# PengjieRen/CaSE_RG

Measured on AMD Instinct MI355X. Metric: train tokens/sec (query+passage) CaSE model, higher is better.
Workload: dtype bf16; 1 GPU; CaSE train step fwd+bwd+allreduce+clip+Adam+EMA, d_model=512, 6 encoder layers, 10 passages x 384 tok, query 64, answer 40, vocab 30522, per-GPU batch 32, dropout on; global_batch=32, parallelism=dp1

## Files before the change

case_rg_amd/_abi.py:

```python
import ctypes as C
import os

import torch

_HERE = os.path.dirname(os.path.abspath(__file__))
LIB_PATH = os.environ.get("CASE_HIP_LIB") or os.path.join(_HERE, "csrc", "libcase_hip.so")

ABI_VERSION = 600
F32, BF16 = 0, 1
WS_ATTENTION_SPLITKV, WS_ATTENTION_BWD, WS_OPTIM_SUMSQ, WS_ENCODER_CHAIN_PACK, WS_GEMM_DW_SLABS = 1, 2, 3, 4, 5
(FEAT_GEMM_256, FEAT_GEMM_SMALL, FEAT_ENCODER_CHAIN, FEAT_ATTN_SCORES, FEAT_ATTN_DECODE, FEAT_OPTIM, FEAT_ATTN_RESIDENT, FEAT_RESERVED_CUS,
 FEAT_GEMM_DW_SLABS, FEAT_DECODER_CHAIN, FEAT_ATTN_DECODE_MQA, FEAT_POINTER_DECODE, FEAT_POINTER_HEAD, FEAT_GEMM_LN, FEAT_STEP_STATE,
 FEAT_INTERACTION, FEAT_ATTN_DECODE_APPEND, FEAT_LINEAR_SKINNY, FEAT_BEAM_DECODE, FEAT_SAMPLE_DECODE, FEAT_POINTER_SCORE, FEAT_CONSENSUS, FEAT_NGRAM_BAN,
 FEAT_NGRAM_COUNTS, FEAT_RANK_METRICS, FEAT_POINTER_HEAD_WIDE, FEAT_DECODE_RULES, FEAT_TOKEN_LABELS,
 FEAT_COPY_ATTRIBUTION, FEAT_METEOR, FEAT_RISK_TRAIN, FEAT_ROUGE_N) = (1 << i for i in range(32))
EPI_BIAS_COL, EPI_BIAS_ROW, EPI_GELU, EPI_RELU = 1, 2, 4, 8
EPI_RESIDUAL, EPI_MUL_DGELU, EPI_MUL_DRELU, EPI_ATOMIC, EPI_DROPOUT = 16, 32, 64, 128, 256

i32, i64, u64, f32, f64, ptr = C.c_int32, C.c_int64, C.c_uint64, C.c_float, C.c_double, C.c_void_p


class GemmDesc(C.Structure):
    _fields_ = [(n, i64) for n in ("M", "N", "K", "lda", "ldb", "ldc", "ld_aux", "batch1", "batch2",
                                   "sa1", "sa2", "sb1", "sb2", "sc1", "sc2", "saux1", "saux2")] + \
# ... 86 lines not shown
    "case_nll_gather_bwd": [ptr, ptr, ptr, ptr, i64, i64, ptr],
    "case_row_argmax": [ptr, ptr, ptr, i64, i64, i64, ptr],
    "case_sentence_compact": [ptr, ptr, ptr, i64, i64, i64, i64, i64, ptr],
    "case_encoder_chain_pack": [ptr, ptr, ptr, ptr, ptr, ptr],
    "case_encoder_chain": [C.POINTER(EncoderChainDesc)] + [ptr] * 14,
    "case_set_reserved_cus": [i32],
    "case_attention_decode_mqa": [ptr, ptr, ptr, ptr, i64, i64, i64, i32, ptr, i64, ptr],
    "case_additive_key_exp": [ptr, ptr, i64, ptr],
    "case_pointer_attend_decode": [ptr] * 11 + [i64, i64, i64, ptr],
    "case_pointer_head_decode": [ptr] * 5 + [i32] + [ptr] * 4 + [i64, i64, i64, ptr],
    "case_pointer_head_beam": [ptr] * 5 + [i32] + [ptr] * 4 + [i64, i64, i64, i32, ptr],
    "case_pointer_head_sample": [ptr] * 5 + [i32] + [ptr] * 7 + [i64, i64, i64, f32, i32, f32, u64, u64, ptr, i64, i64, i64, i32, i32, ptr],
    "case_pointer_head_decode_wide": [ptr] * 5 + [i32] + [ptr] * 4 + [i64, i64, i64, ptr, i64, ptr, i64, i64, i32, i64, ptr],
    "case_pointer_head_beam_wide": [ptr] * 5 + [i32] + [ptr] * 4 + [i64, i64, i64, i32, ptr, i64, ptr, i64, i64, i32, i64, ptr],
    "case_pointer_head_sample_wide": [ptr] * 5 + [i32] + [ptr] * 7 + [i64, i64, i64, f32, i32, f32, u64, u64, ptr, i64, i64, i64, i32, i32,
                                      ptr, i64, ptr, i64, i64, i32, ptr],
    "case_pointer_head_score": [ptr] * 3 + [i64, ptr, ptr, i32, ptr, i64, ptr, ptr, i64, i64, i64, ptr],
    "case_beam_advance": [ptr] * 12 + [i64, i64, i64, i32, i64, ptr],
    "case_pointer_head_decode_ban": [ptr] * 5 + [i32] + [ptr] * 4 + [i64, i64, i64, ptr, i64, i64, i32, i64, ptr],
    "case_pointer_head_beam_ban": [ptr] * 5 + [i32] + [ptr] * 4 + [i64, i64, i64, i32, ptr, i64, i64, i32, i64, ptr],
    "case_pointer_head_sample_ban": [ptr] * 5 + [i32] + [ptr] * 7 + [i64, i64, i64, f32, i32, f32, u64, u64, ptr, i64, i64, i64, i32, i32,
                                     ptr, i64, i64, i32, ptr],
    "case_beam_advance_ban": [ptr] * 12 + [i64, i64, i64, i32, i64, ptr, ptr, i64, ptr],
    "case_ngram_ban": [ptr, ptr, ptr, i64, i64, i64, i64, i32, i64, ptr],
    "case_remove_duplicate_ids": [ptr, ptr, i64, i64, i32, i64, ptr],
    "case_pointer_head_decode_rules": [ptr] * 5 + [i32] + [ptr] * 4 + [i64, i64, i64, ptr, i64, i64, i32, i64] + _RULE + [ptr],
    "case_pointer_head_beam_rules": [ptr] * 5 + [i32] + [ptr] * 4 + [i64, i64, i64, i32, ptr, i64, i64, i32, i64] + _RULE + [ptr],
    "case_pointer_head_sample_rules": [ptr] * 5 + [i32] + [ptr] * 7 + [i64, i64, i64, f32, i32, f32, u64, u64, ptr, i64, i64, i64, i32, i32,
                                       ptr, i64, i64, i32] + _RULE + [ptr],
    "case_pointer_head_decode_wide_rules": [ptr] * 5 + [i32] + [ptr] * 4 + [i64, i64, i64, ptr, i64, ptr, i64, i64, i32, i64] + _RULE + [ptr],
    "case_pointer_head_beam_wide_rules": [ptr] * 5 + [i32] + [ptr] * 4 + [i64, i64, i64, i32, ptr, i64, ptr, i64, i64, i32, i64] + _RULE + [ptr],
    "case_pointer_head_sample_wide_rules": [ptr] * 5 + [i32] + [ptr] * 7 + [i64, i64, i64, f32, i32, f32, u64, u64, ptr, i64, i64, i64, i32, i32,
                                            ptr, i64, ptr, i64, i64, i32] + _RULE + [ptr],
    "case_row_rules": [ptr, ptr, i64, i64, i64] + _RULE + [ptr],
    "case_beam_advance_rules": [ptr] * 12 + [i64, i64, i64, i32, i64, ptr, ptr, i64, f32, ptr],
    "case_beam_gather": [ptr, ptr, i32, ptr, ptr, ptr, i64, i32, i64, i64, i64, ptr],
    "case_beam_backtrack": [ptr] * 8 + [i64, i32, i64, ptr],
    "case_lcs_pairs": [ptr] * 6 + [i64, i64, i64, i64, i64, ptr],
    "case_consensus_pick": [ptr] * 7 + [i64, i64, i64, ptr],
    "case_ngram_counts": [ptr] * 9 + [i64, i64, i64, i64, i64, i32, ptr],
    "case_bleu_scores": [ptr] * 7 + [i64, i64, i64, i32, i32, ptr],
    "case_ngram_distinct": [ptr, ptr, ptr, i64, i64, i32, ptr],
    "case_rouge_n_scores": [ptr] * 9 + [i64, i64, i64, i32, ptr],
    "case_rank_metrics": [ptr] * 8 + [i64, i64, i64, ptr],
    "case_token_labels": [ptr, ptr, ptr, i32, ptr, ptr, i64, i64, i64, i64, i64, i64, ptr],
    "case_token_select": [ptr] * 7 + [i64, i64, i32, ptr],
    "case_copy_attribution": [ptr, ptr, i64, ptr, ptr, i32, ptr, i64, ptr, ptr, i32, ptr, ptr, ptr, ptr, i64, i64, i64, ptr],
    "case_meteor": [ptr] * 5 + [i64, f64, f64, f64] + [ptr] * 5 + [i64, i64, i64, i64, i64, ptr],
    "case_pointer_head_score_stats": [ptr] * 3 + [i64, ptr, ptr, i32, ptr, i64, ptr, ptr, ptr, i64, i64, i64, ptr],
    "case_pointer_head_score_bwd": [ptr] * 3 + [i64, ptr, ptr, i32, ptr, i64] + [ptr] * 6 + [i64, i64, i64, ptr],
    "case_sequence_risk": [ptr] * 4 + [f64] + [ptr] * 3 + [i64, i64, i64, ptr],
    "case_pointer_head_loss": [ptr, i64, ptr, ptr, i64, ptr, ptr, i32, ptr, i64, ptr, ptr, ptr, ptr, i64, i64, i64, ptr],
    "case_pointer_head_loss_bwd": [ptr, i64, ptr, ptr, i64, ptr, ptr, i32, ptr, i64, ptr, ptr, ptr, ptr, i32, ptr, ptr, i64, i64, i64, ptr],
    "case_gemm_ln": [C.POINTER(GemmDesc), ptr, ptr, ptr, f32, ptr, ptr, ptr, ptr, ptr, ptr],
    "case_optim_sumsq": [ptr, ptr, i64, ptr, ptr, ptr],
    "case_optim_adam_ema": [ptr, ptr, i64, ptr, f32, f64, f64, f64, f64, ptr, ptr],
    "case_step_advance": [ptr, u64, f64, f64, ptr],
    "case_interaction_supported": [C.POINTER(InteractionDesc)],
    "case_interaction_fwd": [C.POINTER(InteractionDesc), ptr, ptr, ptr, ptr, ptr, ptr, ptr, ptr, ptr, ptr],
}

OPTIONAL = ("case_pointer_head_loss", "case_pointer_head_loss_bwd")


def _load():
    if not os.path.exists(LIB_PATH):
        raise ImportError(
            "case_rg_amd: %s is missing. Build it with `python -c 'import __graft_entry__ as g; g.build()'` "
            "(or `make -C case_rg_amd/csrc`). There is no CPU or eager fallback." % LIB_PATH)
    lib = C.CDLL(LIB_PATH)
    lib.case_version.restype = C.c_int
    if lib.case_version() != ABI_VERSION:
        raise ImportError("case_rg_amd: %s is ABI generation %d, this package binds %d -- rebuild it (make -C case_rg_amd/csrc)"
                          % (LIB_PATH, lib.case_version(), ABI_VERSION))
    for name, args in SIGNATURES.items():
        if name in OPTIONAL and not hasattr(lib, name):
            continue
        fn = getattr(lib, name)
        fn.argtypes = args
        fn.restype = C.c_int
    lib.case_optim_chunk_elems.restype = C.c_int
    lib.case_optim_chunk_elems.argtypes = []
    lib.case_encoder_chain_packed_bytes.restype = C.c_int64
    lib.case_encoder_chain_packed_bytes.argtypes = []
    lib.case_attention_bwd_scratch_floats.restype = C.c_int64
    lib.case_attention_bwd_scratch_floats.argtypes = [C.POINTER(AttnDesc)]
    lib.case_attention_decode_mqa_workspace.restype = C.c_int64
    lib.case_attention_decode_mqa_workspace.argtypes = [i64, i64, i32]
    lib.case_attention_decode_mqa_splits.restype = C.c_int32
    lib.case_attention_decode_mqa_splits.argtypes = [i64, i64]
    lib.case_abi_features.restype = C.c_uint32
    lib.case_abi_features.argtypes = []
    lib.case_get_reserved_cus.restype = C.c_int
    lib.case_get_reserved_cus.argtypes = []
    lib.case_sizeof_opt_tensor.restype = C.c_int
    lib.case_sizeof_opt_tensor.argtypes = []
    lib.case_sizeof_step_state.restype = C.c_int
    lib.case_sizeof_step_state.argtypes = []
    if lib.case_sizeof_step_state() != C.sizeof(StepState):
        raise ImportError("case_rg_amd: CaseStepState is %d bytes in %s, %d in this binding" % (lib.case_sizeof_step_state(), LIB_PATH, C.sizeof(StepState)))
    lib.case_gemm_dw_slab_bytes.restype = C.c_int64
    lib.case_gemm_dw_slab_bytes.argtypes = [C.POINTER(GemmDesc)]
    lib.case_workspace_bytes.restype = C.c_int64
    lib.case_workspace_bytes.argtypes = [i32, ptr, i64]
    lib.case_gemm_tile_for.restype = C.c_int
    lib.case_gemm_tile_for.argtypes = [C.POINTER(GemmDesc), ptr, ptr, ptr, ptr, ptr, ptr]
    lib.case_last_error.restype = C.c_char_p
    return lib


lib = _load()


def has(name):
    return hasattr(lib, name)
# ... 10 lines not shown
```

case_rg_amd/csrc/attn_pointer.hip:

```cpp
#include "common.h"

namespace {

template <bool FAST>
__device__ __forceinline__ float tanh_t(float x) {
  if constexpr (FAST) {
    const float e = __expf(2.f * x);
    return 1.f - __fdividef(2.f, e + 1.f);
  } else {
    return tanhf(x);
  }
}

constexpr float TANH_PRESCALE = 2.8853900817779268f;
constexpr float EXP2_CLAMP = 62.f;
__device__ __forceinline__ float exp2_factor(float xs) { return __builtin_amdgcn_exp2f(fminf(fmaxf(xs, -EXP2_CLAMP), EXP2_CLAMP)); }
__device__ __forceinline__ float half_sigmoid_prod(float ew, float eu) { return __builtin_amdgcn_rcpf(fmaf(ew, eu, 1.f)); }

constexpr int AJ = 64;
constexpr int AH = 64;
constexpr int ATW = 8;

template <typename T, bool FAST>
__global__ __launch_bounds__(256) void additive_fwd_kernel(const float* __restrict__ wq, const T* __restrict__ uh,
// ... 46 lines not shown
        const int64_t t = tc + wave * ATW + i;
        if (t < Tn) s[(b * Tn + t) * S + j] = FAST ? vsum - 2.f * acc[i] : acc[i];
      }
    }
  }
}

template <typename T, bool FAST, int TT, int NCH>
__global__ __launch_bounds__(256) void additive_fwd_rowwise_kernel(const float* __restrict__ wq, const T* __restrict__ uh,
                                                                   const float* __restrict__ v, float* __restrict__ s,
                                                                   int64_t Tn, int64_t S, int64_t H) {
  constexpr int E = Vec16<T>::N;
  const int64_t b = blockIdx.y;
  const int lane = threadIdx.x & 63;
  const int64_t wave = (int64_t)blockIdx.x * 4 + (threadIdx.x >> 6), nwaves = (int64_t)gridDim.x * 4;
  float wreg[NCH][TT][E], vreg[NCH][E];
#pragma unroll
  for (int c = 0; c < NCH; ++c) {
    const int64_t h0 = ((int64_t)c * 64 + lane) * E;
#pragma unroll
    for (int e = 0; e < E; ++e) {
      vreg[c][e] = h0 < H ? v[h0 + e] : 0.f;
#pragma unroll
      for (int t = 0; t < TT; ++t) wreg[c][t][e] = (h0 < H && t < Tn) ? wq[(b * Tn + t) * H + h0 + e] : 0.f;
    }
  }
  for (int64_t j = wave; j < S; j += nwaves) {
    float acc[TT];
#pragma unroll
    for (int t = 0; t < TT; ++t) acc[t] = 0.f;
#pragma unroll
    for (int c = 0; c < NCH; ++c) {
      const int64_t h0 = ((int64_t)c * 64 + lane) * E;
      if (h0 < H) {
        float u[E];
        Vec16<T>::load(uh + (b * S + j) * H + h0, u);
#pragma unroll
        for (int e = 0; e < E; ++e)
#pragma unroll
          for (int t = 0; t < TT; ++t) acc[t] += vreg[c][e] * tanh_t<FAST>(wreg[c][t][e] + u[e]);
      }
    }
#pragma unroll
    for (int t = 0; t < TT; ++t) {
      const float r = wave_sum(acc[t]);
      if (lane == 0 && t < Tn) s[(b * Tn + t) * S + j] = r;
    }
  }
}

constexpr int BJ = 16;
constexpr int BTC = 32;

template <typename T, bool FAST>
__global__ __launch_bounds__(256) void additive_bwd_uh_kernel(const float* __restrict__ ds, const float* __restrict__ wq,
                                                              const T* __restrict__ uh, const float* __restrict__ v,
                                                              float* __restrict__ d_uh, float* __restrict__ d_v, int64_t Tn,
                                                              int64_t S, int64_t H) {
  __shared__ float DS[BTC][BJ];
  const int64_t b = blockIdx.z, j0 = (int64_t)blockIdx.x * BJ, h = (int64_t)blockIdx.y * 256 + threadIdx.x;
  const bool h_ok = h < H;
  float u[BJ], acc[BJ];
#pragma unroll
  for (int jj = 0; jj < BJ; ++jj) {
    const int64_t j = j0 + jj;
    u[jj] = (h_ok && j < S) ? (FAST ? TANH_PRESCALE : 1.f) * Elem<T>::ld(uh + (b * S + j) * H + h) : 0.f;
    if constexpr (FAST) u[jj] = exp2_factor(u[jj]);
    acc[jj] = 0.f;
  }
  float dv = 0.f, gsum = 0.f;
  for (int64_t tc = 0; tc < Tn; tc += BTC) {
    __syncthreads();
    for (int e = threadIdx.x; e < BTC * BJ; e += 256) {
      const int tt = e / BJ, jj = e % BJ;
      const int64_t t = tc + tt, j = j0 + jj;
      DS[tt][jj] = (t < Tn && j < S) ? ds[(b * Tn + t) * S + j] : 0.f;
    }
    __syncthreads();
    const int tmax = (int)((Tn - tc) < BTC ? (Tn - tc) : BTC);
    for (int tt = 0; tt < tmax; ++tt) {
      float w = h_ok ? (FAST ? TANH_PRESCALE : 1.f) * wq[(b * Tn + tc + tt) * H + h] : 0.f;
      if constexpr (FAST) w = exp2_factor(w);
#pragma unroll
      for (int jj = 0; jj < BJ; ++jj) {
        const float g = DS[tt][jj];
        if constexpr (FAST) {
          const float r = half_sigmoid_prod(w, u[jj]);
          const float gr = g * r;
          acc[jj] += gr - gr * r;
          dv += gr;
          gsum += g;
        } else {
          const float th = tanh_t<FAST>(w + u[jj]);
          acc[jj] += g * (1.f - th * th);
          dv += g * th;
        }
      }
    }
  }
  if (h_ok) {
    const float vh = FAST ? 4.f * v[h] : v[h];
#pragma unroll
    for (int jj = 0; jj < BJ; ++jj) {
      const int64_t j = j0 + jj;
      if (j < S) d_uh[(b * S + j) * H + h] = vh * acc[jj];
    }
    atomicAdd(d_v + h, FAST ? gsum - 2.f * dv : dv);
  }
}

constexpr int CT = 8;
constexpr int CJC = 64;

template <typename T, bool FAST>
__global__ __launch_bounds__(256) void additive_bwd_wq_kernel(const float* __restrict__ ds, const float* __restrict__ wq,
                                                              const T* __restrict__ uh, const float* __restrict__ v,
                                                              float* __restrict__ d_wq, int64_t Tn, int64_t S, int64_t H,
                                                              int tblocks, int64_t j_per) {
  __shared__ float DS[CT][CJC];
  const int64_t b = blockIdx.z, t0 = (int64_t)(blockIdx.x % tblocks) * CT, h = (int64_t)blockIdx.y * 256 + threadIdx.x;
  const int64_t j_begin = (int64_t)(blockIdx.x / tblocks) * j_per, j_end = (j_begin + j_per < S) ? j_begin + j_per : S;
  const bool split = j_per < S;
  const bool h_ok = h < H;
  float w[CT], acc[CT];
#pragma unroll
  for (int tt = 0; tt < CT; ++tt) {
    const int64_t t = t0 + tt;
    w[tt] = (h_ok && t < Tn) ? (FAST ? TANH_PRESCALE : 1.f) * wq[(b * Tn + t) * H + h] : 0.f;
    if constexpr (FAST) w[tt] = exp2_factor(w[tt]);
    acc[tt] = 0.f;
  }
  for (int64_t jc = j_begin; jc < j_end; jc += CJC) {
    __syncthreads();
    for (int e = threadIdx.x; e < CT * CJC; e += 256) {
      const int tt = e / CJC, jj = e % CJC;
      const int64_t t = t0 + tt, j = jc + jj;
      DS[tt][jj] = (t < Tn && j < j_end) ? ds[(b * Tn + t) * S + j] : 0.f;
    }
    __syncthreads();
    const int jmax = (int)((j_end - jc) < CJC ? (j_end - jc) : CJC);
    for (int jj = 0; jj < jmax; ++jj) {
      float u = h_ok ? (FAST ? TANH_PRESCALE : 1.f) * Elem<T>::ld(uh + (b * S + jc + jj) * H + h) : 0.f;
      if constexpr (FAST) u = exp2_factor(u);
#pragma unroll
      for (int tt = 0; tt < CT; ++tt) {
        if constexpr (FAST) {
          const float r = half_sigmoid_prod(w[tt], u);
          const float gr = DS[tt][jj] * r;
          acc[tt] += gr - gr * r;
        } else {
          const float th = tanh_t<FAST>(w[tt] + u);
          acc[tt] += DS[tt][jj] * (1.f - th * th);
        }
      }
    }
  }
  if (h_ok) {
    const float vh = FAST ? 4.f * v[h] : v[h];
#pragma unroll
    for (int tt = 0; tt < CT; ++tt) {
      const int64_t t = t0 + tt;
      if (t < Tn) {
        if (split) atomicAdd(d_wq + (b * Tn + t) * H + h, vh * acc[tt]);
        else d_wq[(b * Tn + t) * H + h] = vh * acc[tt];
      }
    }
  }
}

constexpr float EXP_CLAMP = 43.f;
constexpr int PA_WAVES = 16, PA_H = 512;

__global__ __launch_bounds__(256) void additive_key_exp_kernel(const float* __restrict__ uh, bf16_t* __restrict__ eu, int64_t n8) {
  for (int64_t i = (int64_t)blockIdx.x * 256 + threadIdx.x; i < n8; i += (int64_t)gridDim.x * 256) {
    const float4 a = reinterpret_cast<const float4*>(uh)[2 * i], b = reinterpret_cast<const float4*>(uh)[2 * i + 1];
    const float x[8] = {a.x, a.y, a.z, a.w, b.x, b.y, b.z, b.w};
    float y[8];
#pragma unroll
    for (int e = 0; e < 8; ++e) y[e] = __expf(fminf(fmaxf(2.f * x[e], -EXP_CLAMP), EXP_CLAMP));
    Vec16<bf16_t>::store(eu + 8 * i, y);
  }
}

__device__ __forceinline__ float row_sum4(float r0, float r1, float r2, float r3) {
  const auto a = __builtin_amdgcn_permlane32_swap(__float_as_uint(r0), __float_as_uint(r2), false, false);
  const auto b = __builtin_amdgcn_permlane32_swap(__float_as_uint(r1), __float_as_uint(r3), false, false);
  const float A = __uint_as_float(a[0]) + __uint_as_float(a[1]);
  const float B = __uint_as_float(b[0]) + __uint_as_float(b[1]);
  const auto c = __builtin_amdgcn_permlane16_swap(__float_as_uint(A), __float_as_uint(B), false, false);
  float t = __uint_as_float(c[0]) + __uint_as_float(c[1]);
  t += __uint_as_float(__builtin_amdgcn_update_dpp(0, __float_as_uint(t), 0x128, 0xf, 0xf, false));
  t += __uint_as_float(__builtin_amdgcn_update_dpp(0, __float_as_uint(t), 0x124, 0xf, 0xf, false));
  t += __uint_as_float(__builtin_amdgcn_update_dpp(0, __float_as_uint(t), 0x122, 0xf, 0xf, false));
  t += __uint_as_float(__builtin_amdgcn_update_dpp(0, __float_as_uint(t), 0x121, 0xf, 0xf, false));
  return t;
}

#ifndef CASE_STREAM_DEFAULT_POLICY
typedef unsigned int pa_u32x4 __attribute__((ext_vector_type(4)));
__device__ __forceinline__ uint4 pa_nt_load(const void* p) {
  const pa_u32x4 v = __builtin_nontemporal_load(reinterpret_cast<const pa_u32x4*>(p));
  return make_uint4(v[0], v[1], v[2], v[3]);
}
#define PA_STREAM_LOAD(P) pa_nt_load(P)
#else
#define PA_STREAM_LOAD(P) (*reinterpret_cast<const uint4*>(P))
#endif
__global__ __launch_bounds__(64 * PA_WAVES) void pointer_attend_decode_kernel(
    const float* __restrict__ wq, const float* __restrict__ wq_add, const bf16_t* __restrict__ eu, const float* __restrict__ v, const bf16_t* __restrict__ mem,
    const uint8_t* __restrict__ col_valid, const uint8_t* __restrict__ row_valid, const float* __restrict__ prior, bf16_t* __restrict__ ctx,
    float* __restrict__ p_out, float* __restrict__ copy_out, const int64_t S) {
  extern __shared__ __attribute__((aligned(16))) float pa_smem[];
  float* sc = pa_smem;
  float* red = pa_smem + ((S + 3) & ~(int64_t)3);
  const int lane = threadIdx.x & 63, wave = threadIdx.x >> 6;
  const int64_t b = blockIdx.x;
  const uint8_t* cv = col_valid ? col_valid + b * S : nullptr;
  const bool row_ok = row_valid ? row_valid[b] != 0 : true;
  float ew[8], vv[8];
// ... 1175 lines not shown
                                        int64_t S, int64_t H, int32_t dtype, case_stream_t stream) {
  CASE_REQUIRE(wq && uh && v && s && B > 0 && T > 0 && S > 0 && H > 0 && B < 65536, "case_additive_scores_fwd: bad argument");
  hipStream_t st = (hipStream_t)stream;
  const int ev = dtype == CASE_F32 ? 4 : 8;
  if (T <= 2 && H % ev == 0 && H <= 2 * 64 * ev && (uintptr_t)uh % 16 == 0) {
    const dim3 g((unsigned)((S + 15) / 16 < 64 ? (S + 15) / 16 : 64), (unsigned)B);
    const bool one = H <= 64 * ev;
#define ROWWISE(TY, FAST, TT, NCH) hipLaunchKernelGGL((additive_fwd_rowwise_kernel<TY, FAST, TT, NCH>), g, dim3(256), 0, st, wq, (const TY*)uh, v, s, T, S, H)
    if (dtype == CASE_F32) {
      if (T == 1) { if (one) ROWWISE(float, false, 1, 1); else ROWWISE(float, false, 1, 2); }
      else { if (one) ROWWISE(float, false, 2, 1); else ROWWISE(float, false, 2, 2); }
    } else {
      if (T == 1) { if (one) ROWWISE(bf16_t, true, 1, 1); else ROWWISE(bf16_t, true, 1, 2); }
      else { if (one) ROWWISE(bf16_t, true, 2, 1); else ROWWISE(bf16_t, true, 2, 2); }
    }
#undef ROWWISE
    return case_check_launch("case_additive_scores_fwd");
  }
  const int64_t jb = (S + AJ - 1) / AJ, tchunks = (T + 4 * ATW - 1) / (4 * ATW);
  const dim3 grid((unsigned)jb, (unsigned)B, (unsigned)(jb * B < 512 ? tchunks : 1));
  if (dtype == CASE_F32)
    hipLaunchKernelGGL((additive_fwd_kernel<float, false>), grid, dim3(256), 0, st, wq, (const float*)uh, v, s, T, S, H);
  else
    hipLaunchKernelGGL((additive_fwd_kernel<bf16_t, true>), grid, dim3(256), 0, st, wq, (const bf16_t*)uh, v, s, T, S, H);
  return case_check_launch("case_additive_scores_fwd");
}

extern "C" int case_additive_scores_bwd(const float* ds, const float* wq, const void* uh, const float* v, float* d_wq,
                                        float* d_uh, float* d_v, int64_t B, int64_t T, int64_t S, int64_t H, int32_t dtype,
                                        case_stream_t stream) {
  CASE_REQUIRE(ds && wq && uh && v && d_wq && d_uh && d_v && B > 0 && T > 0 && S > 0 && H > 0 && B < 65536,
               "case_additive_scores_bwd: bad argument");
  const unsigned hb = (unsigned)((H + 255) / 256);
  const int tblocks = (int)((T + CT - 1) / CT);
  const int64_t base_wgs = (int64_t)tblocks * hb * B, j_chunks = (S + CJC - 1) / CJC;
  int64_t sch = base_wgs >= 2048 ? 1 : (2048 + base_wgs - 1) / base_wgs;
  if (sch > j_chunks) sch = j_chunks;
  const int64_t j_per = ((j_chunks + sch - 1) / sch) * CJC;
  sch = (S + j_per - 1) / j_per;
  const dim3 g1((unsigned)((S + BJ - 1) / BJ), hb, (unsigned)B), g2((unsigned)(tblocks * sch), hb, (unsigned)B);
  hipStream_t st = (hipStream_t)stream;
  if (sch > 1 && hipMemsetAsync(d_wq, 0, (size_t)(B * T * H) * sizeof(float), st) != hipSuccess)
    return case_set_error(CASE_E_LAUNCH, "case_additive_scores_bwd: hipMemsetAsync failed");
  if (dtype == CASE_F32) {
    hipLaunchKernelGGL((additive_bwd_uh_kernel<float, false>), g1, dim3(256), 0, st, ds, wq, (const float*)uh, v, d_uh, d_v, T, S, H);
    hipLaunchKernelGGL((additive_bwd_wq_kernel<float, false>), g2, dim3(256), 0, st, ds, wq, (const float*)uh, v, d_wq, T, S, H, tblocks, j_per);
  } else {
    hipLaunchKernelGGL((additive_bwd_uh_kernel<bf16_t, true>), g1, dim3(256), 0, st, ds, wq, (const bf16_t*)uh, v, d_uh, d_v, T, S, H);
    hipLaunchKernelGGL((additive_bwd_wq_kernel<bf16_t, true>), g2, dim3(256), 0, st, ds, wq, (const bf16_t*)uh, v, d_wq, T, S, H, tblocks, j_per);
  }
  return case_check_launch("case_additive_scores_bwd");
}

extern "C" int case_additive_key_exp(const float* uh, void* eu, int64_t n, case_stream_t stream) {
  CASE_REQUIRE(uh && eu && n > 0 && n % 8 == 0 && (uintptr_t)uh % 16 == 0 && (uintptr_t)eu % 16 == 0, "case_additive_key_exp: bad argument");
  hipLaunchKernelGGL(additive_key_exp_kernel, dim3(grid_for(n / 8, 256, 1, 256 * 32)), dim3(256), 0, (hipStream_t)stream, uh,
                     reinterpret_cast<bf16_t*>(eu), n / 8);
  return case_check_launch("case_additive_key_exp");
}

extern "C" int case_pointer_attend_decode(const float* wq, const float* wq_add, const void* eu, const float* v, const void* value, const uint8_t* col_valid,
                                          const uint8_t* row_valid, const float* prior, void* ctx, float* p, float* copy, int64_t B, int64_t S,
                                          int64_t H, case_stream_t stream) {
  CASE_REQUIRE(wq && eu && v && value && ctx && p && B > 0 && S > 0 && B < (1ll << 31) && (copy != nullptr) == (prior != nullptr),
               "case_pointer_attend_decode: bad argument");
  if (H != PA_H || S > 28000)
    return case_set_error(CASE_E_UNSUPPORTED, "case_pointer_attend_decode: built for H = %d and S <= 28000 (run case_additive_scores_fwd + "
                                              "case_softmax_fwd + case_gemm)", PA_H);
  for (const void* q : {(const void*)wq, (const void*)wq_add, eu, (const void*)v, value})
    CASE_REQUIRE((reinterpret_cast<uintptr_t>(q) & 15) == 0, "case_pointer_attend_decode: tensors must be 16-byte aligned");
  const size_t lds = (size_t)(((S + 3) & ~(int64_t)3) + PA_WAVES * PA_H) * sizeof(float);
  static bool attr = false;
  if (!attr) {
    if (hipFuncSetAttribute(reinterpret_cast<const void*>(&pointer_attend_decode_kernel), hipFuncAttributeMaxDynamicSharedMemorySize, 160 * 1024) !=
        hipSuccess)
      return case_set_error(CASE_E_LAUNCH, "case_pointer_attend_decode: cannot reserve LDS");
    attr = true;
  }
  hipLaunchKernelGGL(pointer_attend_decode_kernel, dim3((unsigned)B), dim3(64 * PA_WAVES), lds, (hipStream_t)stream, wq, wq_add,
                     reinterpret_cast<const bf16_t*>(eu), v, reinterpret_cast<const bf16_t*>(value), col_valid, row_valid, prior,
                     reinterpret_cast<bf16_t*>(ctx), p, copy, S);
  return case_check_launch("case_pointer_attend_decode");
}

template <typename Args>
static int pointer_head_fill(Args& a, const char* who, const float* logits, const float* mix_logits, const uint32_t* keys, const float* const* copies,
                             const int64_t* lens, int32_t nmem, int64_t R, int64_t V, int64_t S, int64_t max_v, const char* instead) {
  CASE_REQUIRE(logits && mix_logits && keys && copies && lens && R > 0 && V > 0 && S > 0 && nmem >= 1 && R < (1ll << 31), "%s: bad argument", who);
  if (nmem > PH_MAX_MEM || V > max_v || S > 32768)
    return case_set_error(CASE_E_UNSUPPORTED, "%s: built for <= %d memories, V <= %lld, S <= 32768%s", who, PH_MAX_MEM, (long long)max_v, instead);
  a.logits = logits;
  a.mix_logits = mix_logits;
  a.keys = keys;
  int64_t total = 0;
  for (int m = 0; m < PH_MAX_MEM; ++m) {
    a.copy[m] = m < nmem ? copies[m] : nullptr;
    a.len[m] = m < nmem ? lens[m] : 0;
    total += a.len[m];
    CASE_REQUIRE(m >= nmem || (copies[m] && lens[m] > 0), "%s: null copy weights", who);
  }
  CASE_REQUIRE(total == S, "%s: the memories hold %lld positions, the source map %lld", who, (long long)total, (long long)S);
  a.V = V;
  a.S = S;
  a.nmem = nmem;
  return CASE_OK;
}
// ... 673 lines not shown
```

case_rg_amd/ops.py:

```python
import collections
import math
import ctypes as C
import os

import torch
from torch.autograd import Function

from . import _abi as A
from . import config, paramcache

_DT = {torch.float32: A.F32, torch.bfloat16: A.BF16}


def _code(t):
    try:
        return _DT[t.dtype]
    except KeyError:
        raise TypeError("case_rg_amd: unsupported activation dtype %s" % t.dtype)


_raw_stream, _cur_device = getattr(torch._C, "_cuda_getCurrentRawStream", None), getattr(torch._C, "_cuda_getDevice", None)


def _stream():
# ... 1552 lines not shown
        dEpw = bg(dU, Eqx, Lp, H, Lq, Lq, H, yk=True)
        epw = torch.empty_like(Ep3)
        A.call("case_scale_cols", _ptr(Ep3), _ptr(w3), _ptr(epw), n * Lp, H, _code(Ep3), st)
        dEq_parts.append(bg(dU, epw, Lq, H, Lp, Lq, H, xk=True, yk=True))
        dEp_s = torch.empty_like(Ep3)
        dw1, dw2, dw3 = _zeros_like_shapes(dev, (H,), (H,), (H,))
        A.call("case_scale_cols_bwd", _ptr(dEpw), _ptr(Ep3), _ptr(w3), _ptr(dEp_s), _ptr(dw3), n * Lp, H, _code(Ep3), st)
        dEp_parts.append(dEp_s)
        dap, dcq = dU32.sum(dim=2).reshape(-1).contiguous(), dU32.sum(dim=1).reshape(-1).contiguous()
        dEp_r, dEq_r = torch.empty_like(Ep3), torch.empty_like(Eqx)
        A.call("case_rowdot_bwd", _ptr(dap), _ptr(Ep3), _ptr(w2), _ptr(dEp_r), _ptr(dw2), None, n * Lp, H, _code(Ep3), st)
        A.call("case_rowdot_bwd", _ptr(dcq), _ptr(Eqx), _ptr(w1), _ptr(dEq_r), _ptr(dw1), None, n * Lq, H, _code(Eqx), st)
        dEp_parts.append(dEp_r)
        dEq_parts.append(dEq_r)
        dEp = add_n(dEp_parts).view(Ep.shape)
        dEq = add_n(dEq_parts).view(B, P, Lq, H)
        if nq != P:
            dEq = dEq.float().sum(dim=1, keepdim=True).to(dt)
        dw = torch.cat([dw1, dw2, dw3]).view(w.shape)
        return dEq, dEp, dw, None, None


def interaction_train_supported(Eq, Ep):
    return INTERACTION_TRAIN and interaction_supported(Eq, Ep, False)


class MaxOverPFn(Function):
    @staticmethod
    def forward(ctx, x):
        B, P = x.shape[0], x.shape[1]
        x = x if x.is_contiguous() else x.contiguous()
        inner = x.numel() // (B * P)
        out = torch.empty(B, 1, *x.shape[2:], dtype=x.dtype, device=x.device)
        arg = torch.empty(B * inner, dtype=torch.int32, device=x.device)
        A.call("case_max_over_p_fwd", _ptr(x), _ptr(out), _ptr(arg), B, P, inner, _code(x), _stream())
        ctx.save_for_backward(arg)
        ctx.shape = x.shape
        return out

    @staticmethod
    def backward(ctx, g):
        (arg,) = ctx.saved_tensors
        B, P = ctx.shape[0], ctx.shape[1]
        g = g if g.is_contiguous() else g.contiguous()
        dx = torch.empty(ctx.shape, dtype=g.dtype, device=g.device)
        A.call("case_max_over_p_bwd", _ptr(g), _ptr(arg), _ptr(dx), B, P, dx.numel() // (B * P), _code(g), _stream())
        return dx


def max_over_p(x):
    return MaxOverPFn.apply(x)


class AdditiveScoresFn(Function):
    @staticmethod
    def forward(ctx, wq, uh, v):
        B, T, H = wq.shape
        S = uh.shape[1]
        wq = wq.float().contiguous()
        uh = uh if uh.is_contiguous() else uh.contiguous()
        vv = v.detach().float().contiguous()
        s = torch.empty(B, T, S, dtype=torch.float32, device=wq.device)
        A.call("case_additive_scores_fwd", _ptr(wq), _ptr(uh), _ptr(vv), _ptr(s), B, T, S, H, _code(uh), _stream())
        ctx.save_for_backward(wq, uh, vv)
        return s

    @staticmethod
    def backward(ctx, ds):
        wq, uh, vv = ctx.saved_tensors
        B, T, H = wq.shape
        S = uh.shape[1]
        ds = ds.float().contiguous()
        d_wq = torch.empty_like(wq)
        d_uh = torch.empty(B, S, H, dtype=torch.float32, device=wq.device)
        d_v = _zeros_like_shapes(wq.device, (H,))[0]
        A.call("case_additive_scores_bwd", _ptr(ds), _ptr(wq), _ptr(uh), _ptr(vv), _ptr(d_wq), _ptr(d_uh), _ptr(d_v), B, T, S, H,
               _code(uh), _stream())
        return d_wq, cast(d_uh, uh.dtype), d_v


def additive_scores(wq, uh, v):
    return AdditiveScoresFn.apply(wq, uh, v)


POINTER_FUSED = os.environ.get("CASE_POINTER_FUSED", "auto")
POINTER_FUSED_MIN_BATCH = 96


def pointer_decode_supported(memory):
    return (POINTER_FUSED != "off" and torch.is_tensor(memory) and memory.is_cuda and memory.dtype == torch.bfloat16 and memory.dim() == 3
            and memory.shape[2] == 512 and memory.shape[1] <= 28000 and memory.shape[0] >= POINTER_FUSED_MIN_BATCH
            and not torch.is_grad_enabled()
            and bool(A.lib.case_abi_features() & A.FEAT_POINTER_DECODE))


def additive_key_exp(uh):
    uh = uh.detach()
    uh = uh if uh.is_contiguous() else uh.contiguous()
    eu = torch.empty(uh.shape, dtype=torch.bfloat16, device=uh.device)
    A.call("case_additive_key_exp", _ptr(uh), _ptr(eu), uh.numel(), _stream())
    return eu


def pointer_attend_decode(wq, eu, v, value, col_valid=None, row_valid=None, prior=None, wq_add=None):
    B, S, H = value.shape
    wq = wq.reshape(B, H)
    wq = wq if wq.is_contiguous() else wq.contiguous()
    if wq_add is not None:
        wq_add = wq_add.reshape(B, H)
        if wq_add.dtype != torch.float32 or not wq_add.is_contiguous():
            raise TypeError("pointer_attend_decode: wq_add must be a contiguous f32 [B, H]")
    ctx = torch.empty(B, H, dtype=torch.bfloat16, device=value.device)
    p = torch.empty(B, S, dtype=torch.float32, device=value.device)
    copy = torch.empty_like(p) if prior is not None else None
    if prior is not None:
        prior = prior.reshape(B, S).float()
        prior = prior if prior.is_contiguous() else prior.contiguous()
    A.call("case_pointer_attend_decode", _ptr(wq), _ptr(wq_add), _ptr(eu), _ptr(v), _ptr(value), _ptr(_u8(col_valid)), _ptr(_u8(row_valid)), _ptr(prior),
           _ptr(ctx), _ptr(p), _ptr(copy), B, S, H, _stream())
    return ctx, p, copy


POINTER_HEAD = os.environ.get("CASE_POINTER_HEAD", "auto")
HEAD_LDS_MAX_V = 36000
HEAD_WIDE_MAX_V = 131071
# ... 1118 lines not shown
```

include/case_hip.h:

```cpp
#ifndef CASE_HIP_H
#define CASE_HIP_H

#include <stddef.h>
#include <stdint.h>

#ifdef __cplusplus
extern "C" {
#endif

typedef void* case_stream_t;

typedef enum { CASE_F32 = 0, CASE_BF16 = 1 } case_dtype_t;

enum {
  CASE_OK = 0,
  CASE_E_ARG = -1,
  CASE_E_UNSUPPORTED = -2,
  CASE_E_LAUNCH = -3
};

#define CASE_ABI_VERSION 600
int case_version(void);
enum {
  CASE_FEAT_GEMM_256 = 1u << 0,
// ... 367 lines not shown
int case_remove_duplicate_ids(int64_t* out, int32_t* len, int64_t B, int64_t T, int32_t n, int64_t pad, case_stream_t stream);

int case_lcs_pairs(const int64_t* a, const int32_t* a_len, const int64_t* b, const int32_t* b_len, int32_t* lcs, float* f, int64_t B,
                   int64_t N, int64_t M, int64_t Ta, int64_t Tb, case_stream_t stream);
int case_consensus_pick(const float* f, const float* w, const uint8_t* valid, const int64_t* cand, float* utility, int64_t* index,
                        int64_t* answer, int64_t B, int64_t N, int64_t T, case_stream_t stream);

int case_ngram_counts(const int64_t* a, const int32_t* a_len, const int64_t* b, const int32_t* b_len, int32_t* clip, int32_t* clip_any,
                      int32_t* hit, int32_t* hit_any, int32_t* distinct, int64_t B, int64_t N, int64_t M, int64_t Ta, int64_t Tb,
                      int32_t max_n, case_stream_t stream);
int case_bleu_scores(const int32_t* clip, const int32_t* clip_any, const int32_t* a_len, const int32_t* b_len, float* bleu_pair,
                     double* bleu_any, double* bp, int64_t B, int64_t N, int64_t M, int32_t max_n, int32_t smoothing, case_stream_t stream);

int case_ngram_distinct(const int64_t* b, const int32_t* b_len, int32_t* distinct, int64_t rows, int64_t Tb, int32_t max_n,
                        case_stream_t stream);
int case_rouge_n_scores(const int32_t* hit, const int32_t* hyp_distinct, const int32_t* ref_distinct, const int32_t* b_len, float* f_pair,
                        double* f, double* p, double* r, int32_t* best_ref, int64_t B, int64_t N, int64_t M, int32_t max_n,
                        case_stream_t stream);

int case_rank_metrics(const float* scores, const int32_t* keys, const int32_t* rel, const uint8_t* valid, const int32_t* extra_rel,
                      int32_t* order, double* metrics, int32_t* num_rel, int64_t B, int64_t P, int64_t R, case_stream_t stream);

int case_token_labels(const int64_t* passage, const int64_t* response, const void* freq, int32_t freq_is_i64, float* label, float* weight,
                      int64_t B, int64_t P, int64_t L, int64_t T, int64_t F, int64_t pad, case_stream_t stream);
int case_token_select(const float* values, const uint8_t* valid, const float* scores, const float* labels, int32_t* pos, float* val,
                      int32_t* counts, int64_t B, int64_t S, int32_t K, case_stream_t stream);

int case_copy_attribution(const float* mix_logits, const uint32_t* keys, int64_t rows_per_source, const float* const* copies, const int64_t* lens,
                          int32_t nmem, const int64_t* targets, int64_t pad, const int32_t* seg_start, const int32_t* seg_start_host, int32_t G,
                          float* mass, int32_t* pos, float* pos_mass, int32_t* count, int64_t R, int64_t V, int64_t S, case_stream_t stream);

int case_meteor(const int64_t* a, const int32_t* a_len, const int64_t* b, const int32_t* b_len, const int32_t* classes, int64_t V, double alpha,
                double beta, double gamma, int32_t* counts, float* meteor_pair, double* meteor, int32_t* best_ref, int32_t* align, int64_t B,
                int64_t N, int64_t M, int64_t Ta, int64_t Tb, case_stream_t stream);

int case_pointer_head_score_stats(const float* logits, const float* mix_logits, const uint32_t* keys, int64_t rows_per_source,
                                  const float* const* copies, const int64_t* lens, int32_t nmem, const int64_t* targets, int64_t pad,
                                  float* prob, float* copy, float* stats, int64_t R, int64_t V, int64_t S, case_stream_t stream);
int case_pointer_head_score_bwd(const float* logits, const float* mix_logits, const int64_t* ids, int64_t rows_per_source,
                                const float* const* copies, const int64_t* lens, int32_t nmem, const int64_t* targets, int64_t pad,
                                const float* stats, const float* prob, const float* g, float* d_logits, float* d_mix, float* const* d_copies,
                                int64_t R, int64_t V, int64_t S, case_stream_t stream);
int case_sequence_risk(const float* token_probs, const uint8_t* scored, const float* cost, const uint8_t* valid, double alpha, float* risk,
                       float* q, float* grad_p, int64_t B, int64_t N, int64_t T, case_stream_t stream);

int case_pointer_head_loss(const float* logits, int64_t ld_logits, const float* mix_logits, const uint32_t* keys, int64_t rows_per_source,
                           const float* const* copies, const int64_t* lens, int32_t nmem, const int64_t* targets, int64_t pad, float* prob,
                           float* copy, float* stats, float* nll, int64_t R, int64_t V, int64_t S, case_stream_t stream);
int case_pointer_head_loss_bwd(const float* logits, int64_t ld_logits, const float* mix_logits, const int64_t* ids, int64_t rows_per_source,
                               const float* const* copies, const int64_t* lens, int32_t nmem, const int64_t* targets, int64_t pad,
                               const float* stats, const float* prob, const float* g_nll, void* d_logits, int32_t d_dtype, float* d_mix,
                               float* const* d_copies, int64_t R, int64_t V, int64_t S, case_stream_t stream);

#ifdef __cplusplus
}
#endif
#endif
```

Baseline: 1.344 million tokens/s.

## Fuse additive attention backward into single sweep producing d_wq, d_uh, d_v

Adds a fused backward kernel for additive (tanh) attention scores. It computes d_uh and d_wq in one pass over the score gradients, accumulating per-query partial sums for d_wq in LDS, with atomic adds when the key range is split across blocks. d_uh is now written directly in the input dtype (bf16), which drops the separate fp32 buffer and the cast afterwards. For query lengths above 64 it falls back to the two-kernel path, still with bf16 d_uh output. The risks are extra atomics on d_wq, LDS pressure scaling with T, and the zero-init of d_wq.

```diff
diff --git a/case_rg_amd/_abi.py b/case_rg_amd/_abi.py
--- a/case_rg_amd/_abi.py
+++ b/case_rg_amd/_abi.py
@@ -162,6 +162,7 @@
     "case_sequence_risk": [ptr] * 4 + [f64] + [ptr] * 3 + [i64, i64, i64, ptr],
     "case_pointer_head_loss": [ptr, i64, ptr, ptr, i64, ptr, ptr, i32, ptr, i64, ptr, ptr, ptr, ptr, i64, i64, i64, ptr],
     "case_pointer_head_loss_bwd": [ptr, i64, ptr, ptr, i64, ptr, ptr, i32, ptr, i64, ptr, ptr, ptr, ptr, i32, ptr, ptr, i64, i64, i64, ptr],
+    "case_additive_scores_bwd_fused": [ptr, ptr, ptr, ptr, ptr, ptr, ptr, i64, i64, i64, i64, i32, i64, ptr],
     "case_gemm_ln": [C.POINTER(GemmDesc), ptr, ptr, ptr, f32, ptr, ptr, ptr, ptr, ptr, ptr],
     "case_optim_sumsq": [ptr, ptr, i64, ptr, ptr, ptr],
     "case_optim_adam_ema": [ptr, ptr, i64, ptr, f32, f64, f64, f64, f64, ptr, ptr],
@@ -170,7 +171,7 @@
     "case_interaction_fwd": [C.POINTER(InteractionDesc), ptr, ptr, ptr, ptr, ptr, ptr, ptr, ptr, ptr, ptr],
 }
 
-OPTIONAL = ("case_pointer_head_loss", "case_pointer_head_loss_bwd")
+OPTIONAL = ("case_pointer_head_loss", "case_pointer_head_loss_bwd", "case_additive_scores_bwd_fused")
 
 
 def _load():
diff --git a/case_rg_amd/csrc/attn_pointer.hip b/case_rg_amd/csrc/attn_pointer.hip
--- a/case_rg_amd/csrc/attn_pointer.hip
+++ b/case_rg_amd/csrc/attn_pointer.hip
@@ -122,10 +122,10 @@
 constexpr int BJ = 16;
 constexpr int BTC = 32;
 
-template <typename T, bool FAST>
+template <typename T, bool FAST, typename TO = float>
 __global__ __launch_bounds__(256) void additive_bwd_uh_kernel(const float* __restrict__ ds, const float* __restrict__ wq,
                                                               const T* __restrict__ uh, const float* __restrict__ v,
-                                                              float* __restrict__ d_uh, float* __restrict__ d_v, int64_t Tn,
+                                                              TO* __restrict__ d_uh, float* __restrict__ d_v, int64_t Tn,
                                                               int64_t S, int64_t H) {
   __shared__ float DS[BTC][BJ];
   const int64_t b = blockIdx.z, j0 = (int64_t)blockIdx.x * BJ, h = (int64_t)blockIdx.y * 256 + threadIdx.x;
@@ -173,7 +173,7 @@
 #pragma unroll
     for (int jj = 0; jj < BJ; ++jj) {
       const int64_t j = j0 + jj;
-      if (j < S) d_uh[(b * S + j) * H + h] = vh * acc[jj];
+      if (j < S) Elem<TO>::st(d_uh + (b * S + j) * H + h, vh * acc[jj]);
     }
     atomicAdd(d_v + h, FAST ? gsum - 2.f * dv : dv);
   }
@@ -235,6 +235,92 @@
         else d_wq[(b * Tn + t) * H + h] = vh * acc[tt];
       }
     }
+  }
+}
+
+constexpr int FB_MAX_T = 64;
+constexpr size_t additive_bwd_fused_lds(int64_t Tn) { return (size_t)(Tn * 256 + BTC * BJ + 32) * sizeof(float); }
+
+template <typename T, bool FAST>
+__global__ __launch_bounds__(256) void additive_bwd_fused_kernel(const float* __restrict__ ds, const float* __restrict__ wq,
+                                                                 const T* __restrict__ uh, const float* __restrict__ v,
+                                                                 float* __restrict__ d_wq, T* __restrict__ d_uh, float* __restrict__ d_v,
+                                                                 int64_t Tn, int64_t S, int64_t H, int64_t j_per) {
+  extern __shared__ __attribute__((aligned(16))) float fb_smem[];
+  float* AW = fb_smem;
+  float* DS = AW + Tn * 256;
+  float* red = DS + BTC * BJ;
+  const int64_t b = blockIdx.z, h = (int64_t)blockIdx.y * 256 + threadIdx.x;
+  const int64_t j_begin = (int64_t)blockIdx.x * j_per, j_end = (j_begin + j_per < S) ? j_begin + j_per : S;
+  const bool h_ok = h < H;
+  constexpr float PS = FAST ? TANH_PRESCALE : 1.f;
+  const float vh = h_ok ? (FAST ? 4.f * v[h] : v[h]) : 0.f;
+  for (int64_t t = 0; t < Tn; ++t) AW[t * 256 + threadIdx.x] = 0.f;
+  float dv = 0.f, gpart = 0.f;
+  for (int64_t j0 = j_begin; j0 < j_end; j0 += BJ) {
+    float u[BJ], acc[BJ];
+#pragma unroll
+    for (int jj = 0; jj < BJ; ++jj) {
+      const int64_t j = j0 + jj;
+      u[jj] = (h_ok && j < j_end) ? PS * Elem<T>::ld(uh + (b * S + j) * H + h) : 0.f;
+      if constexpr (FAST) u[jj] = exp2_factor(u[jj]);
+      acc[jj] = 0.f;
+    }
+    for (int64_t tc = 0; tc < Tn; tc += BTC) {
+      __syncthreads();
+      for (int e = threadIdx.x; e < BTC * BJ; e += 256) {
+        const int tt = e / BJ, jj = e % BJ;
+        const int64_t t = tc + tt, j = j0 + jj;
+        const float g = (t < Tn && j < j_end) ? ds[(b * Tn + t) * S + j] : 0.f;
+        DS[tt * BJ + jj] = g;
+        gpart += g;
+      }
+      __syncthreads();
+      const int tmax = (int)((Tn - tc) < BTC ? (Tn - tc) : BTC);
+#pragma unroll 2
+      for (int tt = 0; tt < tmax; ++tt) {
+        float w = h_ok ? PS * wq[(b * Tn + tc + tt) * H + h] : 0.f;
+        if constexpr (FAST) w = exp2_factor(w);
+        float qs = 0.f;
+#pragma unroll
+        for (int jj = 0; jj < BJ; ++jj) {
+          const float g = DS[tt * BJ + jj];
+          if constexpr (FAST) {
+            const float r = half_sigmoid_prod(w, u[jj]);
+            const float gr = g * r;
+            const float q = gr - gr * r;
+            acc[jj] += q;
+            qs += q;
+            dv += gr;
+          } else {
+            const float th = tanh_t<FAST>(w + u[jj]);
+            const float q = g * (1.f - th * th);
+            acc[jj] += q;
+            qs += q;
+            dv += g * th;
+          }
+        }
+        AW[(tc + tt) * 256 + threadIdx.x] += qs;
+      }
+    }
+    if (h_ok) {
+#pragma unroll
+      for (int jj = 0; jj < BJ; ++jj) {
+        const int64_t j = j0 + jj;
+        if (j < j_end) Elem<T>::st(d_uh + (b * S + j) * H + h, vh * acc[jj]);
+      }
+    }
+  }
+  float gsum = 0.f;
+  if constexpr (FAST) gsum = block_sum(gpart, red);
+  if (h_ok) {
+    const bool split = gridDim.x > 1;
+    for (int64_t t = 0; t < Tn; ++t) {
+      const float x = vh * AW[t * 256 + threadIdx.x];
+      if (split) atomicAdd(d_wq + (b * Tn + t) * H + h, x);
+      else d_wq[(b * Tn + t) * H + h] = x;
+    }
+    atomicAdd(d_v + h, FAST ? gsum - 2.f * dv : dv);
   }
 }
 
@@ -1516,6 +1602,58 @@
   return case_check_launch("case_additive_scores_bwd");
 }
 
+extern "C" int case_additive_scores_bwd_fused(const float* ds, const float* wq, const void* uh, const float* v, float* d_wq, void* d_uh,
+                                              float* d_v, int64_t B, int64_t T, int64_t S, int64_t H, int32_t dtype, int64_t j_range,
+                                              case_stream_t stream) {
+  const char* who = "case_additive_scores_bwd_fused";
+  CASE_REQUIRE(ds && wq && uh && v && d_wq && d_uh && d_v && B > 0 && T > 0 && S > 0 && H > 0 && B < 65536 &&
+                   (dtype == CASE_F32 || dtype == CASE_BF16) && j_range >= 0 && j_range % BJ == 0,
+               "%s: bad argument", who);
+  const unsigned hb = (unsigned)((H + 255) / 256);
+  hipStream_t st = (hipStream_t)stream;
+  if (T > FB_MAX_T) {
+    const int tblocks = (int)((T + CT - 1) / CT);
+    const int64_t base_wgs = (int64_t)tblocks * hb * B, j_chunks = (S + CJC - 1) / CJC;
+    int64_t sch = base_wgs >= 2048 ? 1 : (2048 + base_wgs - 1) / base_wgs;
+    if (sch > j_chunks) sch = j_chunks;
+    const int64_t j_per = ((j_chunks + sch - 1) / sch) * CJC;
+    sch = (S + j_per - 1) / j_per;
+    const dim3 g1((unsigned)((S + BJ - 1) / BJ), hb, (unsigned)B), g2((unsigned)(tblocks * sch), hb, (unsigned)B);
+    if (dtype == CASE_F32) {
+      hipLaunchKernelGGL((additive_bwd_uh_kernel<float, false, float>), g1, dim3(256), 0, st, ds, wq, (const float*)uh, v, (float*)d_uh, d_v, T, S, H);
+      hipLaunchKernelGGL((additive_bwd_wq_kernel<float, false>), g2, dim3(256), 0, st, ds, wq, (const float*)uh, v, d_wq, T, S, H, tblocks, j_per);
+    } else {
+      hipLaunchKernelGGL((additive_bwd_uh_kernel<bf16_t, true, bf16_t>), g1, dim3(256), 0, st, ds, wq, (const bf16_t*)uh, v, (bf16_t*)d_uh, d_v, T, S, H);
+      hipLaunchKernelGGL((additive_bwd_wq_kernel<bf16_t, true>), g2, dim3(256), 0, st, ds, wq, (const bf16_t*)uh, v, d_wq, T, S, H, tblocks, j_per);
+    }
+    return case_check_launch(who);
+  }
+  const int64_t base_wgs = (int64_t)hb * B, j_chunks = (S + BJ - 1) / BJ;
+  int64_t ranges = base_wgs >= 4096 ? 1 : (4096 + base_wgs - 1) / base_wgs;
+  if (ranges > j_chunks) ranges = j_chunks;
+  const int64_t j_per = j_range > 0 ? j_range : ((j_chunks + ranges - 1) / ranges) * BJ;
+  ranges = (S + j_per - 1) / j_per;
+  CASE_REQUIRE(ranges < 65536 * 32768ll, "%s: bad argument", who);
+  const dim3 grid((unsigned)ranges, hb, (unsigned)B);
+  const size_t lds = additive_bwd_fused_lds(T);
+  static bool attr = false;
+  if (!attr) {
+    if (hipFuncSetAttribute(reinterpret_cast<const void*>(&additive_bwd_fused_kernel<float, false>), hipFuncAttributeMaxDynamicSharedMemorySize,
+                            (int)additive_bwd_fused_lds(FB_MAX_T)) != hipSuccess ||
+        hipFuncSetAttribute(reinterpret_cast<const void*>(&additive_bwd_fused_kernel<bf16_t, true>), hipFuncAttributeMaxDynamicSharedMemorySize,
+                            (int)additive_bwd_fused_lds(FB_MAX_T)) != hipSuccess)
+      return case_set_error(CASE_E_LAUNCH, "%s: cannot reserve LDS", who);
+    attr = true;
+  }
+  if (dtype == CASE_F32)
+    hipLaunchKernelGGL((additive_bwd_fused_kernel<float, false>), grid, dim3(256), lds, st, ds, wq, (const float*)uh, v, d_wq, (float*)d_uh, d_v, T, S,
+                       H, j_per);
+  else
+    hipLaunchKernelGGL((additive_bwd_fused_kernel<bf16_t, true>), grid, dim3(256), lds, st, ds, wq, (const bf16_t*)uh, v, d_wq, (bf16_t*)d_uh, d_v, T,
+                       S, H, j_per);
+  return case_check_launch(who);
+}
+
 extern "C" int case_additive_key_exp(const float* uh, void* eu, int64_t n, case_stream_t stream) {
   CASE_REQUIRE(uh && eu && n > 0 && n % 8 == 0 && (uintptr_t)uh % 16 == 0 && (uintptr_t)eu % 16 == 0, "case_additive_key_exp: bad argument");
   hipLaunchKernelGGL(additive_key_exp_kernel, dim3(grid_for(n / 8, 256, 1, 256 * 32)), dim3(256), 0, (hipStream_t)stream, uh,
diff --git a/case_rg_amd/ops.py b/case_rg_amd/ops.py
--- a/case_rg_amd/ops.py
+++ b/case_rg_amd/ops.py
@@ -1628,6 +1628,10 @@
     return MaxOverPFn.apply(x)
 
 
+ADDITIVE_BWD = os.environ.get("CASE_ADDITIVE_BWD", "auto")
+ADDITIVE_BWD_J_RANGE = 0
+
+
 class AdditiveScoresFn(Function):
     @staticmethod
     def forward(ctx, wq, uh, v):
@@ -1647,6 +1651,12 @@
         B, T, H = wq.shape
         S = uh.shape[1]
         ds = ds.float().contiguous()
+        if ADDITIVE_BWD != "two_sweep" and A.has("case_additive_scores_bwd_fused"):
+            d_wq, d_v = _zeros_like_shapes(wq.device, tuple(wq.shape), (H,))
+            d_uh = torch.empty(B, S, H, dtype=uh.dtype, device=wq.device)
+            A.call("case_additive_scores_bwd_fused", _ptr(ds), _ptr(wq), _ptr(uh), _ptr(vv), _ptr(d_wq), _ptr(d_uh), _ptr(d_v), B, T, S, H,
+                   _code(uh), ADDITIVE_BWD_J_RANGE, _stream())
+            return d_wq, d_uh, d_v
         d_wq = torch.empty_like(wq)
         d_uh = torch.empty(B, S, H, dtype=torch.float32, device=wq.device)
         d_v = _zeros_like_shapes(wq.device, (H,))[0]
diff --git a/include/case_hip.h b/include/case_hip.h
--- a/include/case_hip.h
+++ b/include/case_hip.h
@@ -443,6 +443,9 @@
                                const float* stats, const float* prob, const float* g_nll, void* d_logits, int32_t d_dtype, float* d_mix,
                                float* const* d_copies, int64_t R, int64_t V, int64_t S, case_stream_t stream);
 
+int case_additive_scores_bwd_fused(const float* ds, const float* wq, const void* uh, const float* v, float* d_wq, void* d_uh, float* d_v,
+                                   int64_t B, int64_t T, int64_t S, int64_t H, int32_t dtype, int64_t j_range, case_stream_t stream);
+
 #ifdef __cplusplus
 }
 #endif
```

Result: slower. 1.315 million tokens/s (-2.2%).
